# mudit1729/dinov2-od

Hardware: AMD Instinct MI355X
Metric: images/sec forward, DINOv2 ViT-B/14 518x518 + 100-query head (higher is better)
Workload: dtype bf16; 1 GPU; ViT-B/14 518x518 bf16, 100 queries, batch 64 per GPU (BASELINE configs[2]'s batch of 64; it fits one GPU, so every GPU runs the whole configuration: weak scaling); global_batch=64, per_gpu_batch=64, image=518, queries=100, parallelism=dp1, hipgraph=True, n_ranks_seen=1, micro_batches=2

## Files before the change

### dinov2_od_amd/csrc/dod_api.hip

```cpp
#include "dod_internal.h"

#include <cstdarg>
#include <cstdio>
#include <atomic>
#include <cstdlib>

using namespace dod;

static std::string g_err;

static int vfail(const dod_handle* h, int code, const char* fmt, va_list ap, int launch_rc = 0) {
  char buf[512];
  const int n = vsnprintf(buf, sizeof buf, fmt, ap);
  if (launch_rc && n >= 0 && (size_t)n < sizeof buf) snprintf(buf + n, sizeof buf - n, " rejected (rc %d)", launch_rc);
  if (h) h->err = buf; else g_err = buf;
  return code;
}
int dod::fail(const dod_handle* h, int code, const char* fmt, ...) {
  va_list ap; va_start(ap, fmt); code = vfail(h, code, fmt, ap); va_end(ap);
  return code;
}
int dod::rejected(const dod_handle* h, int r, const char* fmt, ...) {
  if (!r) return DOD_OK;
  va_list ap; va_start(ap, fmt); const int code = vfail(h, r == 3 ? DOD_ERR_HIP : DOD_ERR_INVALID, fmt, ap, r); va_end(ap);
  return code;
}

static bool check_common(dod_handle* h, int B, int H, int W, int* rc) {
  if (!h) { *rc = fail(nullptr, DOD_ERR_INVALID, "null handle"); return false; }
  if (!h->finalized) { *rc = fail(h, DOD_ERR_STATE, "dod_finalize_weights has not been called"); return false; }
  if (B <= 0) { *rc = fail(h, DOD_ERR_INVALID, "batch must be positive (got %d)", B); return false; }
  if (H < h->cfg.patch || W < h->cfg.patch) { *rc = fail(h, DOD_ERR_INVALID, "image %dx%d smaller than one %dx%d patch", H, W, h->cfg.patch, h->cfg.patch); return false; }
  return true;
}

static std::atomic<int> g_options[DOD_OPT_COUNT] = {{-1}, {-1}, {-1}, {-1}, {-1}, {-1}, {-1}, {-1}, {-1}, {-1}, {-1}};
int dod_option(int which) { return which >= 0 && which < DOD_OPT_COUNT ? g_options[which].load() : -1; }
static const char* const k_option_names[DOD_OPT_COUNT] = {"tailsplit", "dec_fused_split", "mha_chunk_images", "no_fused_patch", "ln_fold", "deterministic", "f32_ksplit",
                                                       "attn_bwd_flash", "epi_regmath", "f32x3_tile", "attn_diet"};

extern "C" {

int dod_test_set_option(const char* name, int value) {
  if (!name) return fail(nullptr, DOD_ERR_INVALID, "null option name");
  for (int i = 0; i < DOD_OPT_COUNT; ++i)
    if (!strcmp(name, k_option_names[i])) { g_options[i].store(value); return DOD_OK; }
  return fail(nullptr, DOD_ERR_INVALID, "unknown test option '%s'", name);
}
long dod_test_counter(const char* name) {
  if (name && !strcmp(name, "tail_splits")) return gemm_tail_split_count();
  if (name && !strcmp(name, "rem_cuts")) return gemm_rem_cut_count();
  if (name && !strcmp(name, "f32_ksplits")) return gemm_f32_ksplit_count();
  if (name && !strcmp(name, "epi_regmath")) return gemm_epi_regmath_count();
  if (name && !strcmp(name, "attn_diet")) return attn_half_tile_count();
  if (name && !strcmp(name, "f32x3_launches")) return gemm_f32x3_count(0);
  if (name && !strcmp(name, "f32x3_wide_launches")) return gemm_f32x3_count(1);
  if (name && !strcmp(name, "optim_launches")) return optim_launch_count();
  if (name && !strcmp(name, "optim_chunk_elems")) return optim_constant(0);
  if (name && !strcmp(name, "optim_table_tensors")) return optim_constant(1);
  if (name && !strcmp(name, "optim_norm_table_tensors")) return optim_constant(2);
  return -1;
}

const char* dod_version(void) { return "dinodet 0.3 (gfx950)"; }
int dod_abi_version(void) { return DOD_ABI_VERSION; }

int dod_device_count(void) {
  int n = 0;
  return hipGetDeviceCount(&n) == hipSuccess ? n : -1;
}

const char* dod_last_error(const dod_handle* h) { return h ? h->err.c_str() : g_err.c_str(); }

int dod_create(const dod_config* cfg, dod_handle** out) {
  if (!cfg || !out) return fail(nullptr, DOD_ERR_INVALID, "null argument");
  const dod_config& c = *cfg;
  if (c.hidden <= 0 || c.layers <= 0 || c.heads <= 0 || c.hidden % c.heads) return fail(nullptr, DOD_ERR_INVALID, "bad backbone dims hidden=%d heads=%d layers=%d", c.hidden, c.heads, c.layers);
  if (c.hidden % 64) return fail(nullptr, DOD_ERR_INVALID, "hidden (%d) must be a multiple of 64", c.hidden);
  {
    const int fm = c.precision == DOD_PREC_FP32 ? 4 : 64;
    if (c.ffn_hidden <= 0 || c.ffn_hidden % fm) return fail(nullptr, DOD_ERR_INVALID, "ffn_hidden (%d) must be a multiple of %d in this precision", c.ffn_hidden, fm);
  }
  if (c.patch <= 0 || c.pos_grid <= 0) return fail(nullptr, DOD_ERR_INVALID, "bad patch/pos_grid");
  if (c.num_queries <= 0 || c.dec_hidden <= 0 || c.dec_heads <= 0 || c.dec_layers <= 0 || c.num_classes <= 0 || c.dim_feedforward <= 0) return fail(nullptr, DOD_ERR_INVALID, "bad decoder dims");
  if (c.dec_hidden % 64 || c.dim_feedforward % 4) return fail(nullptr, DOD_ERR_INVALID, "decoder hidden (%d) must be a multiple of 64, dim_feedforward (%d) of 4", c.dec_hidden, c.dim_feedforward);
  if (c.target_dim && c.target_dim != c.dec_hidden) return fail(nullptr, DOD_ERR_INVALID, "projection dim %d != decoder hidden %d", c.target_dim, c.dec_hidden);
  if (!c.target_dim && c.hidden != c.dec_hidden) return fail(nullptr, DOD_ERR_INVALID, "backbone width %d != decoder hidden %d and no projection", c.hidden, c.dec_hidden);
  if (c.use_deformable && (c.n_points <= 0 || c.n_points > 8)) return fail(nullptr, DOD_ERR_INVALID, "n_points must be 1..8");
  if (c.dec_layers > 64) return fail(nullptr, DOD_ERR_INVALID, "at most 64 decoder layers");
  if (c.precision != DOD_PREC_FP32 && c.precision != DOD_PREC_BF16 && c.precision != DOD_PREC_FP8 && c.precision != DOD_PREC_BF16X3 && c.precision != DOD_PREC_FP16X2) return fail(nullptr, DOD_ERR_INVALID, "unknown precision %d", c.precision);
  dod_handle* h = new (std::nothrow) dod_handle();
  if (!h) return fail(nullptr, DOD_ERR_STATE, "out of host memory");
  h->cfg = c;
  *out = h;
  return DOD_OK;
}

void dod_destroy(dod_handle* h) {
  if (!h) return;
  for (auto& r : h->prof) { (void)hipEventDestroy(r.a); (void)hipEventDestroy(r.b); }
  for (auto e : h->evpool) (void)hipEventDestroy(e);
  for (void* p : h->owned) (void)hipFree(p);
  delete h;
}

int dod_set_weight(dod_handle* h, const char* key, const void* dev_ptr, const int64_t* shape, int ndim, int dtype) {
  if (!h || !key || !dev_ptr || ndim < 0 || ndim > 8 || (ndim && !shape)) return fail(h, DOD_ERR_INVALID, "dod_set_weight: bad argument");
  if (dtype != DOD_F32 && dtype != DOD_BF16) return fail(h, DOD_ERR_INVALID, "dod_set_weight('%s'): dtype %d is neither DOD_F32 nor DOD_BF16", key, dtype);
  std::string k(key);
  if (k.rfind("module.", 0) == 0) k = k.substr(7);
  WRef r; r.raw = dev_ptr; r.dtype = dtype; r.ptr = dtype == DOD_F32 ? (const float*)dev_ptr : nullptr; r.shape.assign(shape, shape + ndim);
  h->w[k] = r;
  h->finalized = false;
  return DOD_OK;
}

int dod_reserve_gemm_scratch(size_t bytes) { return (gemm_tail_reserve(bytes) || gemm_f32_ksplit_reserve()) ? fail(nullptr, DOD_ERR_HIP, "scratch allocation of %zu bytes failed", bytes) : DOD_OK; }

int dod_finalize_weights(dod_handle* h, void* stream) {
  if (!h) return fail(nullptr, DOD_ERR_INVALID, "null handle");
  { static const size_t mb = [] { const char* v = getenv("DINODET_GEMM_SCRATCH_MB"); return v && atoi(v) > 0 ? (size_t)atoi(v) : (size_t)64; }();
    (void)gemm_tail_reserve(mb << 20);
    (void)gemm_f32_ksplit_reserve(); }
  int rc = finalize_impl(h, (hipStream_t)stream);
  if (rc || !h->has_dec) return rc;
  hipStream_t s = (hipStream_t)stream;
  const dod_config& g = h->cfg;
  const size_t Q = g.num_queries, Dd = g.dec_hidden;
  h->l0_tgt = h->l0_proj = nullptr;
  Carver sz(nullptr);
  const size_t bytes = carve_decoder(h, sz, 1, 1, nullptr, false) + 256;
  void* tmp = nullptr;
  float *t0 = nullptr, *p0 = nullptr;
  HIPCHK(h, hipMalloc(&tmp, bytes));
  if (hipMalloc((void**)&t0, Q * Dd * 4) != hipSuccess || (g.use_deformable && hipMalloc((void**)&p0, Q * (size_t)h->ncat * 4) != hipSuccess)) {
    (void)hipFree(tmp); if (t0) (void)hipFree(t0);
    return fail(h, DOD_ERR_HIP, "allocation of the decoder's layer-0 constants failed");
  }
  h->owned.push_back(t0); if (p0) h->owned.push_back(p0);
  Carver cv((void*)(((uintptr_t)tmp + 255) & ~(uintptr_t)255));
  DecWS dw;
  carve_decoder(h, cv, 1, 1, &dw, false);
  rc = decoder_impl(h, nullptr, 1, 1, dw, nullptr, s, true);
  if (!rc) {
    hipError_t e1 = hipMemcpyAsync(t0, dw.tgt, Q * Dd * 4, hipMemcpyDeviceToDevice, s);
    hipError_t e2 = p0 ? hipMemcpyAsync(p0, dw.proj, Q * (size_t)h->ncat * 4, hipMemcpyDeviceToDevice, s) : hipSuccess;
    hipError_t e3 = hipStreamSynchronize(s);
    if (e1 != hipSuccess || e2 != hipSuccess || e3 != hipSuccess) rc = fail(h, DOD_ERR_HIP, "decoder layer-0 constants: %s", hipGetErrorString(e3 != hipSuccess ? e3 : (e1 != hipSuccess ? e1 : e2)));
  } else (void)hipStreamSynchronize(s);
  (void)hipFree(tmp);
  if (rc) return rc;
  h->l0_tgt = t0; h->l0_proj = p0;
  return DOD_OK;
}

int dod_prepare(dod_handle* h, int H, int W, void* stream) {
  if (!h) return fail(nullptr, DOD_ERR_INVALID, "null handle");
  return prepare_impl(h, H, W, (hipStream_t)stream);
}

int dod_num_tokens(const dod_handle* h, int H, int W) { return h ? (H / h->cfg.patch) * (W / h->cfg.patch) + 1 : 0; }

size_t dod_workspace_bytes(const dod_handle* h, int B, int H, int W) {
  if (!h || B <= 0 || H < h->cfg.patch || W < h->cfg.patch) return 0;
  const int N = dod_num_tokens(h, H, W);
  Carver c(nullptr);
  carve_backbone(h, c, B, N, nullptr);
  carve_decoder(h, c, B, N, nullptr, false);
  return c.off + 256;
}

size_t dod_decoder_workspace_bytes(const dod_handle* h, int B, int N) {
  if (!h || B <= 0 || N <= 0) return 0;
  Carver c(nullptr);
  carve_decoder(h, c, B, N, nullptr, true);
  return c.off + 256;
}

int dod_set_tap(dod_handle* h, int stage, float* dst) {
  if (!h) return fail(nullptr, DOD_ERR_INVALID, "null handle");
  if (dst) h->taps[stage] = dst; else h->taps.erase(stage);
  return DOD_OK;
}

int dod_forward(dod_handle* h, const float* pixels, int B, int H, int W, float* det, void* workspace, size_t wsb, void* stream) {
  int rc;
  if (!check_common(h, B, H, W, &rc)) return rc;
  if (!pixels || !det || !workspace) return fail(h, DOD_ERR_INVALID, "null buffer");
  if (wsb < dod_workspace_bytes(h, B, H, W)) return fail(h, DOD_ERR_STATE, "workspace too small: %zu < %zu", wsb, dod_workspace_bytes(h, B, H, W));
  const int N = dod_num_tokens(h, H, W);
  Carver c(align_ws(workspace));
  BbWS bw; DecWS dw;
  carve_backbone(h, c, B, N, &bw);
  carve_decoder(h, c, B, N, &dw, false);
  CARVE_FITS(h, c, workspace, wsb)
  rc = backbone_impl(h, pixels, B, H, W, bw, nullptr, true, (hipStream_t)stream); if (rc) return rc;
  return decoder_impl(h, bw.mem, B, N, dw, det, (hipStream_t)stream);
}

int dod_forward_u8(dod_handle* h, const uint8_t* pixels_hwc, int B, int H, int W, float* det, void* workspace, size_t wsb, void* stream) {
  int rc;
  if (!check_common(h, B, H, W, &rc)) return rc;
  if (!pixels_hwc || !det || !workspace) return fail(h, DOD_ERR_INVALID, "null buffer");
  if (wsb < dod_workspace_bytes(h, B, H, W)) return fail(h, DOD_ERR_STATE, "workspace too small: %zu < %zu", wsb, dod_workspace_bytes(h, B, H, W));
  const int N = dod_num_tokens(h, H, W);
  Carver c(align_ws(workspace));
  BbWS bw; DecWS dw;
// ... 270 lines not shown
```

### dinov2_od_amd/csrc/dod_common.h

```cpp
#pragma once
#include <hip/hip_runtime.h>
#include <stdint.h>
#include <stdlib.h>

typedef __attribute__((ext_vector_type(8))) __bf16 bf16x8;
typedef __attribute__((ext_vector_type(4))) __bf16 bf16x4;
typedef __attribute__((ext_vector_type(2))) __bf16 bf16x2;
typedef __attribute__((ext_vector_type(16))) float f32x16;
typedef __attribute__((ext_vector_type(4))) float f32x4;
typedef __attribute__((ext_vector_type(2))) float f32x2;
typedef unsigned short bf16_t;

#define DOD_WAVE 64

enum { DOD_OPT_TAILSPLIT = 0,
       DOD_OPT_DEC_FUSED_SPLIT,
       DOD_OPT_MHA_CHUNK_IMAGES,
       DOD_OPT_NO_FUSED_PATCH,
       DOD_OPT_LN_FOLD,
       DOD_OPT_DETERMINISTIC,
       DOD_OPT_F32_KSPLIT,
       DOD_OPT_ATTN_BWD_FLASH,
       DOD_OPT_EPI_REGMATH,
       DOD_OPT_F32X3_TILE,
       DOD_OPT_ATTN_DIET,
       DOD_OPT_COUNT };
int dod_option(int which);
long gemm_tail_split_count();
long optim_launch_count();
long optim_constant(int which);
long gemm_rem_cut_count();
long attn_half_tile_count();
long gemm_epi_regmath_count();

#ifdef DINODET_TUNING
#define DOD_TUNE_ENV(name) getenv(name)
#else
#define DOD_TUNE_ENV(name) (static_cast<const char*>(nullptr))
#endif

__device__ __forceinline__ bf16_t f2bf(float f) {
  __bf16 b = (__bf16)f;
  return __builtin_bit_cast(bf16_t, b);
}
__device__ __forceinline__ float bf2f(bf16_t h) {
  return __builtin_bit_cast(float, ((uint32_t)h) << 16);
}
__device__ __forceinline__ uint32_t pack2bf(float lo, float hi) {
  f32x2 v = {lo, hi};
  bf16x2 h = __builtin_convertvector(v, bf16x2);
  return __builtin_bit_cast(uint32_t, h);
}
__device__ __forceinline__ float wave_sum(float v) {
#pragma unroll
  for (int o = 32; o > 0; o >>= 1) v += __shfl_xor(v, o, 64);
  return v;
}
__device__ __forceinline__ float wave_max(float v) {
#pragma unroll
  for (int o = 32; o > 0; o >>= 1) v = fmaxf(v, __shfl_xor(v, o, 64));
  return v;
}
__device__ __forceinline__ unsigned pack4_fp8(float a, float b, float c, float d) {
  int w = __builtin_amdgcn_cvt_pk_fp8_f32(a, b, 0, false);
  w = __builtin_amdgcn_cvt_pk_fp8_f32(c, d, w, true);
  return (unsigned)w;
}
__device__ __forceinline__ unsigned mx_ebyte(float amax) {
  const unsigned b = __float_as_uint(amax * (1.0f / 448.0f));
  unsigned eb = ((b >> 23) & 0xffu) + ((b & 0x7fffffu) ? 1u : 0u);
  eb = eb < 1u ? 1u : (eb > 253u ? 253u : eb);
  return eb;
}
__device__ __forceinline__ float mx_inv_scale(unsigned eb) { return __uint_as_float((254u - eb) << 23); }
__device__ __forceinline__ size_t mx_scale_off(int K, int bi) { return (size_t)(bi & 1) * (K >> 6) + (bi >> 1); }
typedef __attribute__((ext_vector_type(2))) _Float16 f16x2;
typedef __attribute__((ext_vector_type(8))) _Float16 f16x8;
__device__ __forceinline__ float clampf_(float v, float lim) { return __builtin_fminf(__builtin_fmaxf(v, -lim), lim); }
__device__ __forceinline__ void h2_quad(float4 v, float shi, uint2& f16, unsigned& hi8, unsigned& lo8) {
  v.x = clampf_(v.x, 65504.f); v.y = clampf_(v.y, 65504.f); v.z = clampf_(v.z, 65504.f); v.w = clampf_(v.w, 65504.f);
  const f16x2 p0 = {(_Float16)v.x, (_Float16)v.y}, p1 = {(_Float16)v.z, (_Float16)v.w};
  f16.x = __builtin_bit_cast(unsigned, p0); f16.y = __builtin_bit_cast(unsigned, p1);
  const float hx = (float)p0.x, hy = (float)p0.y, hz = (float)p1.x, hw = (float)p1.y;
  const float slo = shi * 2048.0f;
  hi8 = pack4_fp8(clampf_(hx * shi, 448.f), clampf_(hy * shi, 448.f), clampf_(hz * shi, 448.f), clampf_(hw * shi, 448.f));
  lo8 = pack4_fp8(clampf_((v.x - hx) * slo, 448.f), clampf_((v.y - hy) * slo, 448.f), clampf_((v.z - hz) * slo, 448.f), clampf_((v.w - hw) * slo, 448.f));
}
__device__ __forceinline__ size_t h2_off8(int K, int c) { return (size_t)2 * K + (size_t)(c >> 4) * 32 + (c & 15); }

__device__ __forceinline__ float gelu_erf(float x) { return 0.5f * x * (1.0f + erff(x * 0.70710678118654752440f)); }
typedef float f32x2_t __attribute__((ext_vector_type(2)));
__device__ __forceinline__ f32x2_t gelu_fast2(f32x2_t x) {
  f32x2_t ax; ax.x = __builtin_fabsf(x.x); ax.y = __builtin_fabsf(x.y);
  const f32x2_t z = ax * 0.8493218002880191f;
  const f32x2_t d = __builtin_elementwise_fma(z, (f32x2_t)(0.2727374808792225f), (f32x2_t)(1.0f));
  f32x2_t t; t.x = __builtin_amdgcn_rcpf(d.x); t.y = __builtin_amdgcn_rcpf(d.y);
  f32x2_t p = __builtin_elementwise_fma(t, (f32x2_t)(0.5f * 1.061405429f), (f32x2_t)(0.5f * -1.453152027f));
  p = __builtin_elementwise_fma(p, t, (f32x2_t)(0.5f * 1.421413741f));
  p = __builtin_elementwise_fma(p, t, (f32x2_t)(0.5f * -0.284496736f));
  p = __builtin_elementwise_fma(p, t, (f32x2_t)(0.5f * 0.254829592f));
  const f32x2_t nz2 = -z * z;
  f32x2_t e; e.x = __builtin_amdgcn_exp2f(nz2.x); e.y = __builtin_amdgcn_exp2f(nz2.y);
  const f32x2_t q = ax * (t * p);
  const f32x2_t r = __builtin_elementwise_fma(ax, (f32x2_t)(0.5f), x * 0.5f);
  return __builtin_elementwise_fma(-q, e, r);
}
__device__ __forceinline__ void gelu_fast4(float4& v) {
  f32x2_t a = {v.x, v.y}, b = {v.z, v.w};
  a = gelu_fast2(a); b = gelu_fast2(b);
  v.x = a.x; v.y = a.y; v.z = b.x; v.w = b.y;
}
__device__ __forceinline__ float sigmoidf_(float x) { return 1.0f / (1.0f + expf(-x)); }

enum { ACT_NONE = 0, ACT_RELU = 1, ACT_GELU = 2, ACT_SIGMOID = 3 };

struct GemmEpi {
  const float* bias;
  const float* scale;
  const float* resid;
  int ldr;
  float* out_f32;
  bf16_t* out_bf16;
  int ldc;
  int act;
  const float* pos;
  int rows_per_img;
  int out_rows_per_img;
  int out_split;
  const float* a_scale;
  const float* w_scale;
  unsigned char* out_bs;
  const unsigned char* a_bs;
  const unsigned char* w_bs;
  int out_h2;
  const unsigned char* h2_wexp;
  int ksplit;
  int kslice_len;
  long long kslice_stride;
  int glu;
  void* ln_op;
  int ln_op_kind;
  int ln_op_ld;
  float2* ln_part;
  int ln_npart;
  const float2* ln_shift;
  const float2* ln_stats;
  const float* ln_c;
  const float2* ln_part_in;
  float2* ln_stats_out;
  float ln_eps;
};
enum { LNOP_BF16 = 1, LNOP_PAIR = 2, LNOP_H2 = 3 };
inline bool gemm_epi_rows_ok(const GemmEpi& e) {
  return e.rows_per_img == 0 && !e.pos && e.ksplit <= 1 && !e.a_scale && !e.a_bs && !e.out_bs;
}
inline GemmEpi gemm_epi_rows(const GemmEpi& e, int m0) {
  GemmEpi r = e;
  const size_t m = (size_t)m0;
  if (r.resid) r.resid += m * r.ldr;
  if (r.out_f32) r.out_f32 += m * r.ldc;
  if (r.out_bf16) r.out_bf16 += m * r.ldc;
  if (r.ln_op) r.ln_op = reinterpret_cast<char*>(r.ln_op) + m * (size_t)r.ln_op_ld * 2;
  if (r.ln_part) r.ln_part += m * r.ln_npart;
  if (r.ln_shift) r.ln_shift += m;
  if (r.ln_stats) r.ln_stats += m;
  if (r.ln_part_in) r.ln_part_in += m * r.ln_npart;
  if (r.ln_stats_out) r.ln_stats_out += m;
  return r;
}

int launch_gemm_bf16(const bf16_t* A, int lda, const bf16_t* W, int ldw, int M, int N, int K,
                     const GemmEpi& e, hipStream_t s);
int launch_gemm_f32(const float* A, int lda, const float* W, int ldw, int M, int N, int K,
                    const GemmEpi& e, hipStream_t s, bool allow_ksplit = false);
int gemm_f32_ksplit_reserve();
long gemm_f32_ksplit_count();
struct GemmF32X {
  const float* A; const float* W; float* C; const float* bias;
  const float* scale;
  const float* resid;
  int ldr;
  int lda, ldw, ldc, M, N, K;
  long long a_sb, a_sh, w_sb, w_sh, c_sb, c_sh;
  int batch, hb;
  int a_kmajor, w_kmajor;
// ... 81 lines not shown
```

### dinov2_od_amd/csrc/patch_embed.hip

```cpp
#include "dod_common.h"

#define PE_M 128
#define PE_N 128
#define PE_PLANE (128 * 64)

__device__ __forceinline__ int pe_swz(int row, int chunk) { return chunk ^ (((row >> 3) & 1) << 1); }

template <bool X3, bool U8, int P>
__global__ __launch_bounds__(256) void patch_embed_kernel(const void* __restrict__ img_, const bf16_t* __restrict__ Wp, int ldw,
                                                          const float* __restrict__ bias, const float* __restrict__ pos,
                                                          float* __restrict__ out, int B, int H, int W, int gh, int gw, int D) {
  constexpr int p = P;
  extern __shared__ __attribute__((aligned(16))) char smem[];
  constexpr int NPL = X3 ? 4 : 2;
  constexpr int STAGE = NPL * PE_PLANE;
  const int tid = threadIdx.x, lane = tid & 63, wid = tid >> 6;
  const int wu = __builtin_amdgcn_readfirstlane(wid);
  const int wm = wu >> 1, wn = wu & 1;
  const int Np = gh * gw, Mtot = B * Np;
  const int tiles_m = (Mtot + PE_M - 1) / PE_M;
  const int tiles_n = (D + PE_N - 1) / PE_N;
  const int xcd = blockIdx.x & 7, idx = blockIdx.x >> 3;
  const int tn = idx % tiles_n, tm = (idx / tiles_n) * 8 + xcd;
  if (tm >= tiles_m) return;
  const int m0 = tm * PE_M, n0 = tn * PE_N;
  const int nsteps = 3 * (p / 2), kp = nsteps * 32;

  constexpr int NP2 = P / 2;
  unsigned goff[NP2];
  int lofs[NP2];
  size_t cstride, rstride;
  if (U8) { cstride = 1; rstride = (size_t)W * 3; } else { cstride = (size_t)H * W; rstride = (size_t)W; }
#pragma unroll
  for (int i = 0; i < NP2; ++i) {
    const int e = tid + 256 * i;
    const int rr = e / (PE_M * NP2), rem_e = e - rr * (PE_M * NP2), pl = rem_e / NP2, j = 2 * (rem_e - pl * NP2);
    int m = m0 + pl; m = m < Mtot ? m : Mtot - 1;
    const int b = m / Np, rem = m - b * Np, py = rem / gw, px = rem - py * gw;
    if (U8) goff[i] = (unsigned)((((size_t)b * H + (size_t)py * p + rr) * W + (size_t)px * p + j) * 3);
    else goff[i] = (unsigned)((((size_t)b * 3) * H + (size_t)py * p + rr) * W + (size_t)px * p + j);
    const int kq = rr * 16 + j;
    lofs[i] = pl * 64 + pe_swz(pl, kq >> 3) * 16 + (kq & 7) * 2;
  }
  float pv0[P], pv1[P], pv2[P];
  uint4 wA0, wB0, wC0, wD0, wA1, wB1, wC1, wD1, wA2, wB2, wC2, wD2;
  const bf16_t* gWr;
  int wofs0, wofs1;
  {
    const int rl = tid >> 1, hf = tid & 1;
    int rr = n0 + rl; rr = rr < D ? rr : D - 1;
    gWr = Wp + (size_t)rr * ldw + hf * 16;
    wofs0 = rl * 64 + pe_swz(rl, 2 * hf) * 16;
    wofs1 = rl * 64 + pe_swz(rl, 2 * hf + 1) * 16;
  }
#define PE_GLOAD(PV, WA, WB, WC, WD, s_)                                                                    \
  {                                                                                                         \
    const int c_ = (s_) / (p / 2), si_ = (s_) - c_ * (p / 2);                                               \
    const size_t o_ = c_ * cstride + (size_t)(2 * si_) * rstride;                                           \
    _Pragma("unroll") for (int i = 0; i < NP2; ++i) {                                                       \
      if (U8) {                                                                                             \
        const unsigned char* q_ = (const unsigned char*)img_ + goff[i] + o_;                                \
        PV[2 * i] = (float)q_[0] / 255.0f; PV[2 * i + 1] = (float)q_[3] / 255.0f;              \
      } else {                                                                                              \
        const float2 v_ = *reinterpret_cast<const float2*>((const float*)img_ + goff[i] + o_);              \
        PV[2 * i] = v_.x; PV[2 * i + 1] = v_.y;                                                             \
      }                                                                                                     \
    }                                                                                                       \
    const uint4* wp_ = reinterpret_cast<const uint4*>(gWr + (s_) * 32);                                     \
    WA = wp_[0]; WB = wp_[1];                                                                               \
    if (X3) { const uint4* wq_ = reinterpret_cast<const uint4*>(gWr + kp + (s_) * 32); WC = wq_[0]; WD = wq_[1]; } \
  }
#define PE_SWRITE(PV, WA, WB, WC, WD, stage_)                                                               \
  {                                                                                                         \
    char* sa_ = smem + (stage_) * STAGE;                                                                    \
    _Pragma("unroll") for (int i = 0; i < NP2; ++i) {                                                       \
      const unsigned hi_ = pack2bf(PV[2 * i], PV[2 * i + 1]);                                               \
      *reinterpret_cast<unsigned*>(sa_ + lofs[i]) = hi_;                                                    \
      if (X3) *reinterpret_cast<unsigned*>(sa_ + PE_PLANE + lofs[i]) =                                      \
          pack2bf(PV[2 * i] - __uint_as_float(hi_ << 16), PV[2 * i + 1] - __uint_as_float(hi_ & 0xffff0000u)); \
    }                                                                                                       \
    char* sw_ = sa_ + (X3 ? 2 : 1) * PE_PLANE;                                                              \
    *reinterpret_cast<uint4*>(sw_ + wofs0) = WA;                                                            \
    *reinterpret_cast<uint4*>(sw_ + wofs1) = WB;                                                            \
    if (X3) { *reinterpret_cast<uint4*>(sw_ + PE_PLANE + wofs0) = WC; *reinterpret_cast<uint4*>(sw_ + PE_PLANE + wofs1) = WD; } \
  }

  f32x4 acc[4][4];
#pragma unroll
  for (int i = 0; i < 4; ++i)
#pragma unroll
    for (int j = 0; j < 4; ++j) acc[i][j] = f32x4{0.f, 0.f, 0.f, 0.f};
  const int l15 = lane & 15, l4 = lane >> 4;
  int offA[4], offW[4];
#pragma unroll
  for (int i = 0; i < 4; ++i) { const int row = wm * 64 + i * 16 + l15; offA[i] = row * 64 + pe_swz(row, l4) * 16; }
#pragma unroll
  for (int j = 0; j < 4; ++j) { const int row = wn * 64 + j * 16 + l15; offW[j] = (X3 ? 2 : 1) * PE_PLANE + row * 64 + pe_swz(row, l4) * 16; }

  for (int i = tid; i < 2 * STAGE / 16; i += 256) {
    const int st_ = i / (STAGE / 16), o_ = (i - st_ * (STAGE / 16)) * 16;
    if (o_ < (X3 ? 2 : 1) * PE_PLANE) *reinterpret_cast<uint4*>(smem + st_ * STAGE + o_) = make_uint4(0u, 0u, 0u, 0u);
  }
  __syncthreads();
  auto compute = [&](int stage) {
    const char* st = smem + stage * STAGE;
    bf16x8 wh[4], wl[4];
#pragma unroll
    for (int j = 0; j < 4; ++j) {
      wh[j] = *reinterpret_cast<const bf16x8*>(st + offW[j]);
      if (X3) wl[j] = *reinterpret_cast<const bf16x8*>(st + offW[j] + PE_PLANE);
    }
#pragma unroll
    for (int i = 0; i < 4; ++i) {
      const bf16x8 ah = *reinterpret_cast<const bf16x8*>(st + offA[i]);
      bf16x8 al;
      if (X3) al = *reinterpret_cast<const bf16x8*>(st + offA[i] + PE_PLANE);
#pragma unroll
      for (int j = 0; j < 4; ++j) {
        if (X3) {
          acc[i][j] = __builtin_amdgcn_mfma_f32_16x16x32_bf16(wl[j], ah, acc[i][j], 0, 0, 0);
          acc[i][j] = __builtin_amdgcn_mfma_f32_16x16x32_bf16(wh[j], al, acc[i][j], 0, 0, 0);
        }
        acc[i][j] = __builtin_amdgcn_mfma_f32_16x16x32_bf16(wh[j], ah, acc[i][j], 0, 0, 0);
      }
    }
  };
  PE_GLOAD(pv0, wA0, wB0, wC0, wD0, 0)
  PE_GLOAD(pv1, wA1, wB1, wC1, wD1, 1)
  PE_GLOAD(pv2, wA2, wB2, wC2, wD2, 2)
  PE_SWRITE(pv0, wA0, wB0, wC0, wD0, 0)
  __syncthreads();
  for (int s = 0; s < nsteps; s += 3) {
    if (s + 3 < nsteps) PE_GLOAD(pv0, wA0, wB0, wC0, wD0, s + 3)
    compute(s & 1);
    PE_SWRITE(pv1, wA1, wB1, wC1, wD1, (s + 1) & 1)
    __syncthreads();
    if (s + 4 < nsteps) PE_GLOAD(pv1, wA1, wB1, wC1, wD1, s + 4)
    compute((s + 1) & 1);
    PE_SWRITE(pv2, wA2, wB2, wC2, wD2, (s + 2) & 1)
    __syncthreads();
    if (s + 5 < nsteps) PE_GLOAD(pv2, wA2, wB2, wC2, wD2, s + 5)
    compute((s + 2) & 1);
    if (s + 3 < nsteps) PE_SWRITE(pv0, wA0, wB0, wC0, wD0, (s + 3) & 1)
    __syncthreads();
  }
  const int N = Np + 1;
#pragma unroll
  for (int i = 0; i < 4; ++i) {
    const int m = m0 + wm * 64 + i * 16 + l15;
    if (m >= Mtot) continue;
    const int b = m / Np, rem = m - b * Np;
    float* orow = out + ((size_t)b * N + 1 + rem) * D;
    const float* prow = pos + (size_t)(1 + rem) * D;
#pragma unroll
    for (int j = 0; j < 4; ++j) {
      const int n = n0 + wn * 64 + j * 16 + 4 * l4;
      if (n >= D) continue;
      const float4 bv = *reinterpret_cast<const float4*>(bias + n), pp = *reinterpret_cast<const float4*>(prow + n);
      const f32x4 a = acc[i][j];
      *reinterpret_cast<float4*>(orow + n) = make_float4(a[0] + bv.x + pp.x, a[1] + bv.y + pp.y, a[2] + bv.z + pp.z, a[3] + bv.w + pp.w);
    }
  }
}

__global__ void patch_pack_kernel(const float* __restrict__ W, int D, int p, bf16_t* __restrict__ out, int x3) {
  const int kp = 3 * (p / 2) * 32;
  const size_t total = (size_t)D * kp;
  for (size_t idx = (size_t)blockIdx.x * blockDim.x + threadIdx.x; idx < total; idx += (size_t)gridDim.x * blockDim.x) {
    const int n = (int)(idx / kp), k = (int)(idx - (size_t)n * kp);
    const int s = k >> 5, kk = k & 31, r = kk >> 4, j = kk & 15;
    const int c = s / (p / 2), si = s - c * (p / 2);
    const float v = j < p ? W[(((size_t)n * 3 + c) * p + (2 * si + r)) * p + j] : 0.f;
    const bf16_t hi = f2bf(v);
    if (x3) {
      out[(size_t)n * 2 * kp + k] = hi;
      out[(size_t)n * 2 * kp + kp + k] = f2bf(v - bf2f(hi));
    } else {
      out[idx] = hi;
    }
  }
}

int launch_patch_pack(const float* W, int D, int p, bf16_t* out, int x3, hipStream_t s) {
  if (p < 2 || p > 16 || (p & 1)) return 2;
  const size_t total = (size_t)D * 3 * (p / 2) * 32;
  hipLaunchKernelGGL(patch_pack_kernel, dim3((unsigned)((total + 255) / 256 < 4096 ? (total + 255) / 256 : 4096)), dim3(256), 0, s, W, D, p, out, x3);
  return hipGetLastError() == hipSuccess ? 0 : 3;
}

int launch_patch_embed(const void* img, int u8, int B, int H, int W, int p, const bf16_t* Wp, int x3, const float* bias, const float* pos,
                       float* out, int D, hipStream_t s) {
  if ((p != 14 && p != 16) || D % 4 != 0 || B <= 0 || (!u8 && (W & 1))) return 2;
  const int gh = H / p, gw = W / p;
  if (gh <= 0 || gw <= 0) return 2;
  if ((size_t)B * 3 * H * W >= 0xffffffffull) return 2;
  const int kp = 3 * (p / 2) * 32, ldw = x3 ? 2 * kp : kp;
  const int tiles = ((((B * gh * gw) + PE_M - 1) / PE_M + 7) / 8 * 8) * ((D + PE_N - 1) / PE_N);
  const int lds = 2 * (x3 ? 4 : 2) * PE_PLANE;
#define PE_LAUNCH(X3_, U8_, P_) hipLaunchKernelGGL((patch_embed_kernel<X3_, U8_, P_>), dim3(tiles), dim3(256), lds, s, img, Wp, ldw, bias, pos, out, B, H, W, gh, gw, D)
  if (p == 14) {
    if (x3) { if (u8) PE_LAUNCH(true, true, 14); else PE_LAUNCH(true, false, 14); }
    else { if (u8) PE_LAUNCH(false, true, 14); else PE_LAUNCH(false, false, 14); }
  } else {
    if (x3) { if (u8) PE_LAUNCH(true, true, 16); else PE_LAUNCH(true, false, 16); }
    else { if (u8) PE_LAUNCH(false, true, 16); else PE_LAUNCH(false, false, 16); }
  }
#undef PE_LAUNCH
  return hipGetLastError() == hipSuccess ? 0 : 3;
}
```

Baseline: 2605 images/s.

## Add wide 384-column patch-embed tile with six waves to reuse image tiles

Templates the patch-embed kernel on the number of column waves so a block can cover 384 output channels with 768 threads. The gathered image tile is then loaded and converted once for three times as many columns. The wide variant is picked automatically when there are enough tiles to fill the CUs and the split-precision path is off. It also adds a test option and a counter. The trade-off is a larger LDS footprint and block size, which means fewer resident blocks, plus new ragged-pass indexing in the gather.

After: 2610 images/s, median of 6. About the same (+0.2%).

```diff
diff --git a/dinov2_od_amd/csrc/dod_api.hip b/dinov2_od_amd/csrc/dod_api.hip
--- a/dinov2_od_amd/csrc/dod_api.hip
+++ b/dinov2_od_amd/csrc/dod_api.hip
@@ -34,10 +34,10 @@
   return true;
 }
 
-static std::atomic<int> g_options[DOD_OPT_COUNT] = {{-1}, {-1}, {-1}, {-1}, {-1}, {-1}, {-1}, {-1}, {-1}, {-1}, {-1}};
+static std::atomic<int> g_options[DOD_OPT_COUNT] = {{-1}, {-1}, {-1}, {-1}, {-1}, {-1}, {-1}, {-1}, {-1}, {-1}, {-1}, {-1}};
 int dod_option(int which) { return which >= 0 && which < DOD_OPT_COUNT ? g_options[which].load() : -1; }
 static const char* const k_option_names[DOD_OPT_COUNT] = {"tailsplit", "dec_fused_split", "mha_chunk_images", "no_fused_patch", "ln_fold", "deterministic", "f32_ksplit",
-                                                       "attn_bwd_flash", "epi_regmath", "f32x3_tile", "attn_diet"};
+                                                       "attn_bwd_flash", "epi_regmath", "f32x3_tile", "attn_diet", "patch_tile"};
 
 extern "C" {
 
@@ -53,6 +53,7 @@
   if (name && !strcmp(name, "f32_ksplits")) return gemm_f32_ksplit_count();
   if (name && !strcmp(name, "epi_regmath")) return gemm_epi_regmath_count();
   if (name && !strcmp(name, "attn_diet")) return attn_half_tile_count();
+  if (name && !strcmp(name, "patch_wide")) return patch_wide_count();
   if (name && !strcmp(name, "f32x3_launches")) return gemm_f32x3_count(0);
   if (name && !strcmp(name, "f32x3_wide_launches")) return gemm_f32x3_count(1);
   if (name && !strcmp(name, "optim_launches")) return optim_launch_count();
diff --git a/dinov2_od_amd/csrc/dod_common.h b/dinov2_od_amd/csrc/dod_common.h
--- a/dinov2_od_amd/csrc/dod_common.h
+++ b/dinov2_od_amd/csrc/dod_common.h
@@ -24,6 +24,7 @@
        DOD_OPT_EPI_REGMATH,
        DOD_OPT_F32X3_TILE,
        DOD_OPT_ATTN_DIET,
+       DOD_OPT_PATCH_TILE,
        DOD_OPT_COUNT };
 int dod_option(int which);
 long gemm_tail_split_count();
@@ -31,6 +32,7 @@
 long optim_constant(int which);
 long gemm_rem_cut_count();
 long attn_half_tile_count();
+long patch_wide_count();
 long gemm_epi_regmath_count();
 
 #ifdef DINODET_TUNING
diff --git a/dinov2_od_amd/csrc/patch_embed.hip b/dinov2_od_amd/csrc/patch_embed.hip
--- a/dinov2_od_amd/csrc/patch_embed.hip
+++ b/dinov2_od_amd/csrc/patch_embed.hip
@@ -1,22 +1,24 @@
 #include "dod_common.h"
+#include <atomic>
 
 #define PE_M 128
-#define PE_N 128
 #define PE_PLANE (128 * 64)
 
 __device__ __forceinline__ int pe_swz(int row, int chunk) { return chunk ^ (((row >> 3) & 1) << 1); }
 
-template <bool X3, bool U8, int P>
-__global__ __launch_bounds__(256) void patch_embed_kernel(const void* __restrict__ img_, const bf16_t* __restrict__ Wp, int ldw,
+template <bool X3, bool U8, int P, int WN>
+__global__ __launch_bounds__(128 * WN) void patch_embed_kernel(const void* __restrict__ img_, const bf16_t* __restrict__ Wp, int ldw,
                                                           const float* __restrict__ bias, const float* __restrict__ pos,
                                                           float* __restrict__ out, int B, int H, int W, int gh, int gw, int D) {
   constexpr int p = P;
   extern __shared__ __attribute__((aligned(16))) char smem[];
-  constexpr int NPL = X3 ? 4 : 2;
-  constexpr int STAGE = NPL * PE_PLANE;
+  constexpr int T = 128 * WN, PE_N = 64 * WN;
+  constexpr int NA = X3 ? 2 : 1;
+  constexpr int PE_WPLANE = PE_N * 64;
+  constexpr int STAGE = NA * (PE_PLANE + PE_WPLANE);
   const int tid = threadIdx.x, lane = tid & 63, wid = tid >> 6;
   const int wu = __builtin_amdgcn_readfirstlane(wid);
-  const int wm = wu >> 1, wn = wu & 1;
+  const int wm = wu / WN, wn = wu % WN;
   const int Np = gh * gw, Mtot = B * Np;
   const int tiles_m = (Mtot + PE_M - 1) / PE_M;
   const int tiles_n = (D + PE_N - 1) / PE_N;
@@ -26,14 +28,16 @@
   const int m0 = tm * PE_M, n0 = tn * PE_N;
   const int nsteps = 3 * (p / 2), kp = nsteps * 32;
 
-  constexpr int NP2 = P / 2;
-  unsigned goff[NP2];
-  int lofs[NP2];
+  constexpr int NP2 = P / 2, PAIRS = PE_M * P, NPASS = (PAIRS + T - 1) / T;
+  static_assert((NPASS - 1) * T < PAIRS && NPASS >= 2, "ragged last pass repeats the one before it");
+  unsigned goff[NPASS];
+  int lofs[NPASS];
   size_t cstride, rstride;
   if (U8) { cstride = 1; rstride = (size_t)W * 3; } else { cstride = (size_t)H * W; rstride = (size_t)W; }
 #pragma unroll
-  for (int i = 0; i < NP2; ++i) {
-    const int e = tid + 256 * i;
+  for (int i = 0; i < NPASS; ++i) {
+    int e = tid + T * i;
+    if (e >= PAIRS) e -= T;
     const int rr = e / (PE_M * NP2), rem_e = e - rr * (PE_M * NP2), pl = rem_e / NP2, j = 2 * (rem_e - pl * NP2);
     int m = m0 + pl; m = m < Mtot ? m : Mtot - 1;
     const int b = m / Np, rem = m - b * Np, py = rem / gw, px = rem - py * gw;
@@ -42,8 +46,8 @@
     const int kq = rr * 16 + j;
     lofs[i] = pl * 64 + pe_swz(pl, kq >> 3) * 16 + (kq & 7) * 2;
   }
-  float pv0[P], pv1[P], pv2[P];
-  uint4 wA0, wB0, wC0, wD0, wA1, wB1, wC1, wD1, wA2, wB2, wC2, wD2;
+  float pv0[2 * NPASS], pv1[2 * NPASS], pv2[2 * NPASS];
+  uint4 w0a, w0b, w0c, w0d, w1a, w1b, w1c, w1d, w2a, w2b, w2c, w2d;
   const bf16_t* gWr;
   int wofs0, wofs1;
   {
@@ -53,11 +57,11 @@
     wofs0 = rl * 64 + pe_swz(rl, 2 * hf) * 16;
     wofs1 = rl * 64 + pe_swz(rl, 2 * hf + 1) * 16;
   }
-#define PE_GLOAD(PV, WA, WB, WC, WD, s_)                                                                    \
+#define PE_GLOAD(PV, K, s_)                                                                                 \
   {                                                                                                         \
     const int c_ = (s_) / (p / 2), si_ = (s_) - c_ * (p / 2);                                               \
     const size_t o_ = c_ * cstride + (size_t)(2 * si_) * rstride;                                           \
-    _Pragma("unroll") for (int i = 0; i < NP2; ++i) {                                                       \
+    _Pragma("unroll") for (int i = 0; i < NPASS; ++i) {                                                       \
       if (U8) {                                                                                             \
         const unsigned char* q_ = (const unsigned char*)img_ + goff[i] + o_;                                \
         PV[2 * i] = (float)q_[0] / 255.0f; PV[2 * i + 1] = (float)q_[3] / 255.0f;              \
@@ -67,22 +71,22 @@
       }                                                                                                     \
     }                                                                                                       \
     const uint4* wp_ = reinterpret_cast<const uint4*>(gWr + (s_) * 32);                                     \
-    WA = wp_[0]; WB = wp_[1];                                                                               \
-    if (X3) { const uint4* wq_ = reinterpret_cast<const uint4*>(gWr + kp + (s_) * 32); WC = wq_[0]; WD = wq_[1]; } \
-  }
-#define PE_SWRITE(PV, WA, WB, WC, WD, stage_)                                                               \
+    w##K##a = wp_[0]; w##K##b = wp_[1];                                                                     \
+    if (X3) { const uint4* wq_ = reinterpret_cast<const uint4*>(gWr + kp + (s_) * 32); w##K##c = wq_[0]; w##K##d = wq_[1]; } \
+  }
+#define PE_SWRITE(PV, K, stage_)                                                                            \
   {                                                                                                         \
     char* sa_ = smem + (stage_) * STAGE;                                                                    \
-    _Pragma("unroll") for (int i = 0; i < NP2; ++i) {                                                       \
+    _Pragma("unroll") for (int i = 0; i < NPASS; ++i) {                                                       \
       const unsigned hi_ = pack2bf(PV[2 * i], PV[2 * i + 1]);                                               \
       *reinterpret_cast<unsigned*>(sa_ + lofs[i]) = hi_;                                                    \
       if (X3) *reinterpret_cast<unsigned*>(sa_ + PE_PLANE + lofs[i]) =                                      \
           pack2bf(PV[2 * i] - __uint_as_float(hi_ << 16), PV[2 * i + 1] - __uint_as_float(hi_ & 0xffff0000u)); \
     }                                                                                                       \
-    char* sw_ = sa_ + (X3 ? 2 : 1) * PE_PLANE;                                                              \
-    *reinterpret_cast<uint4*>(sw_ + wofs0) = WA;                                                            \
-    *reinterpret_cast<uint4*>(sw_ + wofs1) = WB;                                                            \
-    if (X3) { *reinterpret_cast<uint4*>(sw_ + PE_PLANE + wofs0) = WC; *reinterpret_cast<uint4*>(sw_ + PE_PLANE + wofs1) = WD; } \
+    char* sw_ = sa_ + NA * PE_PLANE;                                                                        \
+    *reinterpret_cast<uint4*>(sw_ + wofs0) = w##K##a;                                                       \
+    *reinterpret_cast<uint4*>(sw_ + wofs1) = w##K##b;                                                       \
+    if (X3) { *reinterpret_cast<uint4*>(sw_ + PE_WPLANE + wofs0) = w##K##c; *reinterpret_cast<uint4*>(sw_ + PE_WPLANE + wofs1) = w##K##d; } \
   }
 
   f32x4 acc[4][4];
@@ -95,11 +99,11 @@
 #pragma unroll
   for (int i = 0; i < 4; ++i) { const int row = wm * 64 + i * 16 + l15; offA[i] = row * 64 + pe_swz(row, l4) * 16; }
 #pragma unroll
-  for (int j = 0; j < 4; ++j) { const int row = wn * 64 + j * 16 + l15; offW[j] = (X3 ? 2 : 1) * PE_PLANE + row * 64 + pe_swz(row, l4) * 16; }
-
-  for (int i = tid; i < 2 * STAGE / 16; i += 256) {
-    const int st_ = i / (STAGE / 16), o_ = (i - st_ * (STAGE / 16)) * 16;
-    if (o_ < (X3 ? 2 : 1) * PE_PLANE) *reinterpret_cast<uint4*>(smem + st_ * STAGE + o_) = make_uint4(0u, 0u, 0u, 0u);
+  for (int j = 0; j < 4; ++j) { const int row = wn * 64 + j * 16 + l15; offW[j] = NA * PE_PLANE + row * 64 + pe_swz(row, l4) * 16; }
+
+  for (int i = tid; i < 2 * NA * PE_PLANE / 16; i += T) {
+    const int st_ = i / (NA * PE_PLANE / 16), o_ = (i - st_ * (NA * PE_PLANE / 16)) * 16;
+    *reinterpret_cast<uint4*>(smem + st_ * STAGE + o_) = make_uint4(0u, 0u, 0u, 0u);
   }
   __syncthreads();
   auto compute = [&](int stage) {
@@ -108,7 +112,7 @@
 #pragma unroll
     for (int j = 0; j < 4; ++j) {
       wh[j] = *reinterpret_cast<const bf16x8*>(st + offW[j]);
-      if (X3) wl[j] = *reinterpret_cast<const bf16x8*>(st + offW[j] + PE_PLANE);
+      if (X3) wl[j] = *reinterpret_cast<const bf16x8*>(st + offW[j] + PE_WPLANE);
     }
 #pragma unroll
     for (int i = 0; i < 4; ++i) {
@@ -125,23 +129,23 @@
       }
     }
   };
-  PE_GLOAD(pv0, wA0, wB0, wC0, wD0, 0)
-  PE_GLOAD(pv1, wA1, wB1, wC1, wD1, 1)
-  PE_GLOAD(pv2, wA2, wB2, wC2, wD2, 2)
-  PE_SWRITE(pv0, wA0, wB0, wC0, wD0, 0)
+  PE_GLOAD(pv0, 0, 0)
+  PE_GLOAD(pv1, 1, 1)
+  PE_GLOAD(pv2, 2, 2)
+  PE_SWRITE(pv0, 0, 0)
   __syncthreads();
   for (int s = 0; s < nsteps; s += 3) {
-    if (s + 3 < nsteps) PE_GLOAD(pv0, wA0, wB0, wC0, wD0, s + 3)
+    if (s + 3 < nsteps) PE_GLOAD(pv0, 0, s + 3)
     compute(s & 1);
-    PE_SWRITE(pv1, wA1, wB1, wC1, wD1, (s + 1) & 1)
+    PE_SWRITE(pv1, 1, (s + 1) & 1)
     __syncthreads();
-    if (s + 4 < nsteps) PE_GLOAD(pv1, wA1, wB1, wC1, wD1, s + 4)
+    if (s + 4 < nsteps) PE_GLOAD(pv1, 1, s + 4)
     compute((s + 1) & 1);
-    PE_SWRITE(pv2, wA2, wB2, wC2, wD2, (s + 2) & 1)
+    PE_SWRITE(pv2, 2, (s + 2) & 1)
     __syncthreads();
-    if (s + 5 < nsteps) PE_GLOAD(pv2, wA2, wB2, wC2, wD2, s + 5)
+    if (s + 5 < nsteps) PE_GLOAD(pv2, 2, s + 5)
     compute((s + 2) & 1);
-    if (s + 3 < nsteps) PE_SWRITE(pv0, wA0, wB0, wC0, wD0, (s + 3) & 1)
+    if (s + 3 < nsteps) PE_SWRITE(pv0, 0, (s + 3) & 1)
     __syncthreads();
   }
   const int N = Np + 1;
@@ -188,6 +192,18 @@
   return hipGetLastError() == hipSuccess ? 0 : 3;
 }
 
+static std::atomic<long> g_patch_wide{0};
+long patch_wide_count() { return g_patch_wide.load(); }
+
+static int pe_cu_count() {
+  static int cus[16] = {};
+  int dev = 0, n = 0;
+  (void)hipGetDevice(&dev);
+  if (dev < 0 || dev >= 16) dev = 0;
+  if (!cus[dev]) cus[dev] = hipDeviceGetAttribute(&n, hipDeviceAttributeMultiprocessorCount, dev) == hipSuccess && n > 0 ? n : 256;
+  return cus[dev];
+}
+
 int launch_patch_embed(const void* img, int u8, int B, int H, int W, int p, const bf16_t* Wp, int x3, const float* bias, const float* pos,
                        float* out, int D, hipStream_t s) {
   if ((p != 14 && p != 16) || D % 4 != 0 || B <= 0 || (!u8 && (W & 1))) return 2;
@@ -195,16 +211,20 @@
   if (gh <= 0 || gw <= 0) return 2;
   if ((size_t)B * 3 * H * W >= 0xffffffffull) return 2;
   const int kp = 3 * (p / 2) * 32, ldw = x3 ? 2 * kp : kp;
-  const int tiles = ((((B * gh * gw) + PE_M - 1) / PE_M + 7) / 8 * 8) * ((D + PE_N - 1) / PE_N);
-  const int lds = 2 * (x3 ? 4 : 2) * PE_PLANE;
-#define PE_LAUNCH(X3_, U8_, P_) hipLaunchKernelGGL((patch_embed_kernel<X3_, U8_, P_>), dim3(tiles), dim3(256), lds, s, img, Wp, ldw, bias, pos, out, B, H, W, gh, gw, D)
-  if (p == 14) {
-    if (x3) { if (u8) PE_LAUNCH(true, true, 14); else PE_LAUNCH(true, false, 14); }
-    else { if (u8) PE_LAUNCH(false, true, 14); else PE_LAUNCH(false, false, 14); }
-  } else {
-    if (x3) { if (u8) PE_LAUNCH(true, true, 16); else PE_LAUNCH(true, false, 16); }
-    else { if (u8) PE_LAUNCH(false, true, 16); else PE_LAUNCH(false, false, 16); }
-  }
+  const int tiles_m8 = (((B * gh * gw) + PE_M - 1) / PE_M + 7) / 8 * 8;
+  const int opt = dod_option(DOD_OPT_PATCH_TILE);
+  const bool wide = !x3 && opt != 0 && (opt == 1 || ((B * gh * gw + PE_M - 1) / PE_M) * ((D + 383) / 384) >= pe_cu_count());
+  const int tile_n = wide ? 384 : 128;
+  const int tiles = tiles_m8 * ((D + tile_n - 1) / tile_n);
+  const int lds = 2 * (x3 ? 2 : 1) * (PE_PLANE + tile_n * 64);
+#define PE_LAUNCH(X3_, U8_, P_, WN_) hipLaunchKernelGGL((patch_embed_kernel<X3_, U8_, P_, WN_>), dim3(tiles), dim3(128 * WN_), lds, s, img, Wp, ldw, bias, pos, out, B, H, W, gh, gw, D)
+#define PE_LAUNCH_P(P_)                                                                          \
+  if (x3) { if (u8) PE_LAUNCH(true, true, P_, 2); else PE_LAUNCH(true, false, P_, 2); }          \
+  else if (wide) { if (u8) PE_LAUNCH(false, true, P_, 6); else PE_LAUNCH(false, false, P_, 6); } \
+  else { if (u8) PE_LAUNCH(false, true, P_, 2); else PE_LAUNCH(false, false, P_, 2); }
+  if (p == 14) { PE_LAUNCH_P(14) } else { PE_LAUNCH_P(16) }
+#undef PE_LAUNCH_P
 #undef PE_LAUNCH
+  if (wide) ++g_patch_wide;
   return hipGetLastError() == hipSuccess ? 0 : 3;
 }
```
